# ipc-sim/IPC

Hardware: NVIDIA H100
Metric: newton_iteration_ms_assembly_ccd (lower is better)
Workload: dtype f64

## Files before the change

ipc_b200/csrc/abi.h:

```cpp
#pragma once
#include "../../include/ipcgpu.h"
#include "context.h"
#include <cstddef>
#include <string>

#define CK(call)                                                                                  \
    do {                                                                                          \
        cudaError_t e_ = (call);                                                                  \
        if (e_ != cudaSuccess) {                                                                  \
            ctx->err = std::string(#call) + ": " + cudaGetErrorString(e_);                        \
            return IPCGPU_ERR_CUDA;                                                               \
        }                                                                                         \
    } while (0)
#define REQUIRE(cond, code, msg)                                                                  \
    do {                                                                                          \
        if (!(cond)) {                                                                            \
            ctx->err = (msg);                                                                     \
            return (code);                                                                        \
        }                                                                                         \
    } while (0)
#define ALLOC(buf, count) REQUIRE((buf).reserve(count), IPCGPU_ERR_CUDA, "cudaMalloc failed for " #buf)

static inline int nblk(long long n, int b) { return (int)((n + b - 1) / b); }

enum Chain { kSerial, kStepBound, kDerivative };

inline int join_deriv(ipcgpu_ctx* ctx)
{
    if (!ctx->deriv_open) return IPCGPU_OK;
    ctx->deriv_open = false;
    CK(cudaEventRecord(ctx->ev_deriv_done, ctx->deriv));
    CK(cudaStreamWaitEvent(ctx->stream, ctx->ev_deriv_done, 0));
    return IPCGPU_OK;
}

inline int enter(ipcgpu_ctx* ctx, Chain chain)
{
    CK(cudaSetDevice(ctx->device));
    if (chain == kStepBound) return IPCGPU_OK;
    if (chain == kSerial || ctx->nranks > 1 || ctx->profiling) return join_deriv(ctx);
    if (ctx->deriv_open) return IPCGPU_OK;
    CK(cudaEventRecord(ctx->ev_deriv_fork, ctx->stream));
    CK(cudaStreamWaitEvent(ctx->deriv, ctx->ev_deriv_fork, 0));
    ctx->deriv_open = true;
    return IPCGPU_OK;
}
#define ENTER(chain)                                                                              \
    do {                                                                                          \
        int re_ = enter(ctx, (chain));                                                            \
        if (re_) return re_;                                                                      \
    } while (0)

int join_copy_stream(ipcgpu_ctx* ctx);
int fetch_iter_state(ipcgpu_ctx* ctx);
int sync_pattern_mirror(ipcgpu_ctx* ctx);
int flag_status(ipcgpu_ctx* ctx, unsigned mask);
void set_local(ipcgpu_ctx* ctx, unsigned bits, bool local);
int energy_result(ipcgpu_ctx* ctx, int slot, double* E, bool fetch = false, unsigned check = 0);
int energy_tail(ipcgpu_ctx* ctx, int slot, const double* partials, int n_partials, double scale, cudaEvent_t pe, double* E, bool fetch = false,
    unsigned check = 0);
int gradient_roundtrip_begin(ipcgpu_ctx* ctx, const double* g_in);
int gradient_roundtrip_end(ipcgpu_ctx* ctx, double* g_out);
int hessian_begin(ipcgpu_ctx* ctx, Chain chain, const double* a_inout);
int hessian_end(ipcgpu_ctx* ctx, double* a_inout, unsigned check);

int nccl_sum(ipcgpu_ctx* ctx, double* buf, size_t n, const char* what);
int nccl_sum(ipcgpu_ctx* ctx, int* buf, size_t n, const char* what);
int nccl_min_u64(ipcgpu_ctx* ctx, unsigned long long* word);
int nccl_all_gather(ipcgpu_ctx* ctx, const int4* send, int4* recv, size_t n, const char* what);
void nccl_comm_destroy(ipcgpu_ctx* ctx);

int build_maps(ipcgpu_ctx* ctx);
void owned_value_range(ipcgpu_ctx* ctx);
int ensure_offsets(ipcgpu_ctx* ctx);
int upload_dir(ipcgpu_ctx* ctx, const double* p);

int timestep_prepare(ipcgpu_ctx* ctx, ipcgpu::DynamicsArgs* p);
// ... 56 lines not shown
```

ipc_b200/csrc/api.cu:

```cuda
#include "abi.h"
#include <cstring>

using namespace ipcgpu;

int join_copy_stream(ipcgpu_ctx* ctx)
{
    if (!ctx->copy_pending) return IPCGPU_OK;
    CK(cudaEventRecord(ctx->ev_copy_join, ctx->copy));
    CK(cudaStreamWaitEvent(ctx->stream, ctx->ev_copy_join, 0));
    ctx->copy_pending = false;
    return IPCGPU_OK;
}

int fetch_iter_state(ipcgpu_ctx* ctx)
{
    {
        int rcj = join_copy_stream(ctx);
        if (rcj) return rcj;
    }
    CK(cudaMemcpyAsync(ctx->h_iter, ctx->iter.p, sizeof(IterState), cudaMemcpyDeviceToHost, ctx->stream));
    CK(cudaStreamSynchronize(ctx->stream));
    return IPCGPU_OK;
}

// ... 127 lines not shown

int hessian_begin(ipcgpu_ctx* ctx, Chain chain, const double* a_inout)
{
    REQUIRE(ctx->nnz > 0, IPCGPU_ERR_STATE, "ipcgpu_set_csr first");
    ENTER(a_inout ? kSerial : chain);
    return a_inout ? upload_values(ctx, a_inout) : IPCGPU_OK;
}
int hessian_end(ipcgpu_ctx* ctx, double* a_inout, unsigned check)
{
    if (!a_inout) return IPCGPU_OK;
    int rc = download_values(ctx, a_inout);
    if (rc || !check || (rc = fetch_iter_state(ctx))) return rc;
    return flag_status(ctx, check);
}

extern "C" {

int ipcgpu_create(int device, ipcgpu_ctx** out)
{
    if (!out) return IPCGPU_ERR_ARG;
    *out = nullptr;
    int ndev = 0;
    if (cudaGetDeviceCount(&ndev) != cudaSuccess || ndev == 0) return IPCGPU_ERR_CUDA;
    if (device < 0 || device >= ndev) return IPCGPU_ERR_ARG;
    if (cudaSetDevice(device) != cudaSuccess) return IPCGPU_ERR_CUDA;
    ipcgpu_ctx* ctx = new ipcgpu_ctx();
    ctx->device = device;
    void* hi = nullptr;
    if (cudaDeviceGetStreamPriorityRange(&ctx->prio_low, &ctx->prio_high) != cudaSuccess
        || cudaStreamCreateWithPriority(&ctx->stream, cudaStreamNonBlocking, ctx->prio_high) != cudaSuccess
        || cudaStreamCreateWithPriority(&ctx->deriv, cudaStreamNonBlocking, ctx->prio_low) != cudaSuccess
        || cudaEventCreateWithFlags(&ctx->ev_deriv_fork, cudaEventDisableTiming) != cudaSuccess
        || cudaEventCreateWithFlags(&ctx->ev_deriv_done, cudaEventDisableTiming) != cudaSuccess
        || cudaStreamCreateWithFlags(&ctx->side, cudaStreamNonBlocking) != cudaSuccess || cudaEventCreateWithFlags(&ctx->ev_inputs, cudaEventDisableTiming) != cudaSuccess
        || cudaEventCreateWithFlags(&ctx->ev_join, cudaEventDisableTiming) != cudaSuccess || cudaEventCreateWithFlags(&ctx->ev_scatter, cudaEventDisableTiming) != cudaSuccess
        || cudaMallocHost(&ctx->staging, sizeof(HostStaging)) != cudaSuccess
        || cudaMallocHost(&hi, sizeof(IterState)) != cudaSuccess || !ctx->flag.reserve(4) || !ctx->packed_scalars.reserve(kPackedScalars) || !ctx->iter.reserve(1)
        || cudaMemsetAsync(ctx->iter.p, 0, sizeof(IterState), ctx->stream) != cudaSuccess) {
        ipcgpu_destroy(ctx);
        return IPCGPU_ERR_CUDA;
    }
    ctx->h_iter = static_cast<IterState*>(hi);
    std::memset(ctx->h_iter, 0, sizeof(IterState));
    step_set(ctx->iter.p, 1.0, ctx->stream);
    *out = ctx;
    return IPCGPU_OK;
}

void ipcgpu_destroy(ipcgpu_ctx* ctx)
{
    if (!ctx) return;
    cudaSetDevice(ctx->device);
    if (ctx->side) cudaStreamSynchronize(ctx->side);
    if (ctx->deriv) cudaStreamSynchronize(ctx->deriv);
    if (ctx->copy) {
        cudaStreamSynchronize(ctx->copy);
        cudaStreamDestroy(ctx->copy);
        cudaEventDestroy(ctx->ev_copy_fork);
        cudaEventDestroy(ctx->ev_copy_join);
    }
    if (ctx->stream) cudaStreamSynchronize(ctx->stream);
    for (auto& r : ctx->graphs) {
        if (r.exec) cudaGraphExecDestroy(r.exec);
        if (r.graph) cudaGraphDestroy(r.graph);
    }
    if (ctx->ev_inputs) cudaEventDestroy(ctx->ev_inputs);
    if (ctx->ev_join) cudaEventDestroy(ctx->ev_join);
    if (ctx->ev_scatter) cudaEventDestroy(ctx->ev_scatter);
    if (ctx->side) cudaStreamDestroy(ctx->side);
    if (ctx->ev_deriv_fork) cudaEventDestroy(ctx->ev_deriv_fork);
    if (ctx->ev_deriv_done) cudaEventDestroy(ctx->ev_deriv_done);
    if (ctx->deriv) cudaStreamDestroy(ctx->deriv);
    for (cudaStream_t s : ctx->cond_streams)
        if (s) cudaStreamDestroy(s);
    for (auto& v : ctx->prof)
        for (auto& pr : v) {
            cudaEventDestroy(pr.first);
            cudaEventDestroy(pr.second);
        }
    if (ctx->timer_a) cudaEventDestroy(ctx->timer_a);
    if (ctx->timer_b) cudaEventDestroy(ctx->timer_b);
    nccl_comm_destroy(ctx);
    if (ctx->stream) cudaStreamDestroy(ctx->stream);
    if (ctx->staging) cudaFreeHost(ctx->staging);
    if (ctx->h_iter) cudaFreeHost(ctx->h_iter);
    delete ctx;
}

const char* ipcgpu_last_error(const ipcgpu_ctx* ctx) { return ctx ? ctx->err.c_str() : "null context"; }
int ipcgpu_host_alloc(void** ptr, uint64_t bytes) { return cudaMallocHost(ptr, bytes) == cudaSuccess ? IPCGPU_OK : IPCGPU_ERR_CUDA; }
int ipcgpu_host_free(void* ptr) { return cudaFreeHost(ptr) == cudaSuccess ? IPCGPU_OK : IPCGPU_ERR_CUDA; }
int ipcgpu_sync(ipcgpu_ctx* ctx)
{
    ENTER(kSerial);
    int rcj = join_copy_stream(ctx);
    if (rcj) return rcj;
    CK(cudaStreamSynchronize(ctx->stream));
    return IPCGPU_OK;
}
uint64_t ipcgpu_launch_count(const ipcgpu_ctx* ctx) { return ctx ? ctx->launches : 0; }

int ipcgpu_allreduce_grad_hess(ipcgpu_ctx* ctx, int with_gradient, int with_hessian)
{
    if (ctx->nranks <= 1) return IPCGPU_OK;
// ... 210 lines not shown
```

ipc_b200/csrc/api_contact.cu:

```cuda
#include "abi.h"
#include <algorithm>
#include <cmath>
#include <vector>

using namespace ipcgpu;

extern "C" {

int ipcgpu_set_surface(ipcgpu_ctx* ctx, int nSV, const int* SVI, int nSE, const int* SE, int nSF, const int* SF, const int* vCoDim)
{
    ENTER(kSerial);
    ++ctx->epoch;
    REQUIRE(ctx->nV > 0, IPCGPU_ERR_STATE, "ipcgpu_set_mesh first");
    REQUIRE(nSV >= 0 && nSE >= 0 && nSF >= 0 && (nSV == 0 || SVI) && (nSE == 0 || SE) && (nSF == 0 || SF), IPCGPU_ERR_ARG, "ipcgpu_set_surface: bad arguments");
    for (int i = 0; i < nSV; ++i) REQUIRE(SVI[i] >= 0 && SVI[i] < ctx->nV, IPCGPU_ERR_ARG, "SVI out of range");
    for (int i = 0; i < 2 * nSE; ++i) REQUIRE(SE[i] >= 0 && SE[i] < ctx->nV, IPCGPU_ERR_ARG, "SFEdges out of range");
    for (size_t i = 0; i < (size_t)3 * nSF; ++i) REQUIRE(SF[i] >= 0 && SF[i] < ctx->nV, IPCGPU_ERR_ARG, "SF out of range");
    ctx->nSV = nSV; ctx->nSE = nSE; ctx->nSF = nSF;
    bool ok = ctx->SVI.upload(SVI, std::max(nSV, 0), ctx->stream) && ctx->SE.upload(SE, (size_t)2 * nSE, ctx->stream) && ctx->SF.upload(SF, (size_t)3 * nSF, ctx->stream);
    REQUIRE(ok, IPCGPU_ERR_CUDA, "surface upload failed");
    ctx->has_codim = vCoDim != nullptr;
    if (vCoDim) REQUIRE(ctx->vCoDim.upload(vCoDim, ctx->nV, ctx->stream), IPCGPU_ERR_CUDA, "codim upload failed");
    CK(cudaStreamSynchronize(ctx->stream));
    ctx->h_SVI.assign(SVI, SVI + nSV);
// ... 162 lines not shown
}

int ipcgpu_ccd_stats_timing(ipcgpu_ctx* ctx, uint64_t* longest_pair_cycles, uint64_t* total_pair_cycles)
{
    if (longest_pair_cycles) *longest_pair_cycles = ctx->ccd.last_longest_cycles;
    if (total_pair_cycles) *total_pair_cycles = ctx->ccd.last_total_cycles;
    return IPCGPU_OK;
}

int ipcgpu_set_exchange_capacity(ipcgpu_ctx* ctx, int pairs_per_rank)
{
    ENTER(kSerial);
    ++ctx->epoch;
    REQUIRE(pairs_per_rank > 0, IPCGPU_ERR_ARG, "capacity must be positive");
    ctx->exchange_capacity = pairs_per_rank;
    if (ctx->surface_ready) return contact_alloc(ctx);
    return IPCGPU_OK;
}

int ipcgpu_set_pair_capacity(ipcgpu_ctx* ctx, int capacity)
{
    ENTER(kSerial);
    ++ctx->epoch;
    REQUIRE(capacity > 0, IPCGPU_ERR_ARG, "capacity must be positive");
    ctx->pair_capacity = capacity;
    if (ctx->surface_ready) return contact_alloc(ctx);
    return IPCGPU_OK;
}

int ipcgpu_constraint_set(ipcgpu_ctx* ctx, double dHat, int getPTEE, int* nC, int* nPara, int* nCand)
{
    REQUIRE(ctx->surface_ready, IPCGPU_ERR_STATE, "ipcgpu_set_surface first");
    REQUIRE(dHat > 0.0, IPCGPU_ERR_ARG, "dHat must be positive");
    ENTER(kSerial);
    int rc = contact_constraint_set(ctx, dHat, getPTEE, nC, nPara, nCand);
    ctx->lists_local = (rc == 0) && ctx->partition_contact && ctx->nranks > 1;
    ctx->cw.lists_global = false;
    if (rc == 0 && ctx->lists_local) {
        ContactWork& w = ctx->cw;
        contact_pack_lists(ctx);
        cudaEvent_t pe = ctx->prof_begin(IPCGPU_STAGE_ALLREDUCE);
        const int r = nccl_all_gather(ctx, w.xsend.p, w.xrecv.p, w.xstride, "ncclAllGather(pair lists) failed");
        ctx->prof_end(pe);
        if (r) return r;
        contact_unpack_lists(ctx);
        w.lists_global = true;
        CK(cudaGetLastError());
    }
    ctx->mark_inputs();
    return rc;
}

int ipcgpu_set_canonical_order(ipcgpu_ctx* ctx, int enable)
{
    ENTER(kSerial);
    ++ctx->epoch;
    ctx->canonical_order = enable != 0;
    return IPCGPU_OK;
}

int ipcgpu_set_contact_partition(ipcgpu_ctx* ctx, int enable)
{
    ENTER(kSerial);
    ++ctx->epoch;
    ctx->partition_contact = enable != 0;
    return IPCGPU_OK;
}
// ... 106 lines not shown
    if ((rc = sync_pattern_mirror(ctx))) return rc;
    if (changed) *changed = ctx->pat_changed_host;
    if (nnz) *nnz = ctx->nnz;
    return flag_status(ctx, 1u << FLAG_PATTERN_CAPACITY);
}

int ipcgpu_pattern_info(ipcgpu_ctx* ctx, int* changed, int64_t* nnz, uint64_t* version)
{
    REQUIRE(ctx->device_pattern, IPCGPU_ERR_STATE, "ipcgpu_enable_device_pattern first");
    ENTER(kSerial);
    int rc = sync_pattern_mirror(ctx);
    if (rc) return rc;
    if (changed) *changed = ctx->pat_changed_host;
    if (nnz) *nnz = ctx->nnz;
    if (version) *version = ctx->pat_seen_version;
    return IPCGPU_OK;
}

int ipcgpu_get_pattern(ipcgpu_ctx* ctx, int* ia, int* ja)
{
    REQUIRE(ctx->n_rows > 0, IPCGPU_ERR_STATE, "no pattern: ipcgpu_set_csr or ipcgpu_enable_device_pattern first");
    ENTER(kSerial);
    int rc = sync_pattern_mirror(ctx);
    if (rc) return rc;
    if (ia) CK(cudaMemcpyAsync(ia, ctx->ia.p, ((size_t)ctx->n_rows + 1) * sizeof(int), cudaMemcpyDeviceToHost, ctx->stream));
    if (ja) CK(cudaMemcpyAsync(ja, ctx->ja.p, (size_t)ctx->nnz * sizeof(int), cudaMemcpyDeviceToHost, ctx->stream));
    CK(cudaStreamSynchronize(ctx->stream));
    return IPCGPU_OK;
}

int ipcgpu_barrier_energy(ipcgpu_ctx* ctx, double dHat, double kappa, double* E)
{
    REQUIRE(ctx->surface_ready, IPCGPU_ERR_STATE, "ipcgpu_set_surface first");
    ENTER(kSerial);
    BarrierArgs p = barrier_args(ctx, dHat, kappa, 0);
    cudaEvent_t pe = ctx->prof_begin(IPCGPU_STAGE_BARRIER);
    barrier_energy(p, ctx->cw.bpartials.p, &ctx->iter.p->flags[FLAG_NONPOSITIVE_DISTANCE], ctx->stream);
    return energy_tail(ctx, kEnergyBarrier, ctx->cw.bpartials.p, barrier_energy_blocks(), kappa, pe, E, true, 1u << FLAG_NONPOSITIVE_DISTANCE);
}

int ipcgpu_barrier_gradient(ipcgpu_ctx* ctx, double dHat, double kappa, double* g_inout)
{
    REQUIRE(ctx->surface_ready, IPCGPU_ERR_STATE, "ipcgpu_set_surface first");
    const BarrierArgs p = barrier_args(ctx, dHat, kappa, 0);
    return gradient_call(ctx, kDerivative, g_inout, [&](cudaStream_t st) { barrier_gradient(p, ctx->g.p, st); });
}

int ipcgpu_evaluate_constraints(ipcgpu_ctx* ctx, double* val, int n)
{
    REQUIRE(ctx->surface_ready, IPCGPU_ERR_STATE, "ipcgpu_set_surface first");
    ENTER(kSerial);
    ContactWork& w = ctx->cw;
    if (w.nC < 0) {
        int rc = contact_sync_counts(ctx);
        if (rc) return rc;
    }
    REQUIRE(n == w.nC && (val || n == 0), IPCGPU_ERR_ARG, "ipcgpu_evaluate_constraints: n must be the size of the active set on this context");
    ALLOC(w.bval, (size_t)std::max(w.cap, 1));
    BarrierArgs p = barrier_args(ctx, 1.0, 1.0, 0);
    p.cs = w.act.p; p.nC = w.counters.p + 0;
    evaluate_constraints(p, w.bval.p, ctx->stream);
    ++ctx->launches;
    CK(cudaGetLastError());
    if (n) CK(cudaMemcpyAsync(val, w.bval.p, (size_t)n * sizeof(double), cudaMemcpyDeviceToHost, ctx->stream));
    CK(cudaStreamSynchronize(ctx->stream));
    return IPCGPU_OK;
}
// ... 206 lines not shown
```

ipc_b200/csrc/api_mesh.cu:

```cuda
#include "abi.h"
#include <algorithm>
#include <cmath>
#include <numeric>
#include <vector>

using namespace ipcgpu;

int build_maps(ipcgpu_ctx* ctx)
{
    const int nT = ctx->nT, nV = ctx->nV;
    const std::vector<int>& T = ctx->h_T;
    ctx->t_begin = (int)((int64_t)nT * ctx->rank / ctx->nranks);
    ctx->t_end = (int)((int64_t)nT * (ctx->rank + 1) / ctx->nranks);
    std::vector<int64_t> cum(nV + 1, 0);
    for (size_t i = 0; i < (size_t)4 * nT; ++i) ++cum[T[i] + 1];
    for (int v = 0; v < nV; ++v) cum[v + 1] += cum[v];
    auto boundary = [&](int r) -> int {
        if (r <= 0) return 0;
        if (r >= ctx->nranks) return nV;
        const int64_t target = cum[nV] * r / ctx->nranks;
        return (int)(std::lower_bound(cum.begin(), cum.end(), target) - cum.begin());
    };
    const int vb = std::min(boundary(ctx->rank), nV), ve = std::max(vb, std::min(boundary(ctx->rank + 1), nV));
    ctx->v_begin = vb;
// ... 306 lines not shown
        e_part = ctx->e_partials2.p;
    }
    elastic_grad_hess(ctx->eargs(), coef, projectSPD, need_g, need_h, ctx->gcont.p, ctx->hblk.p, st, e_part);
    ctx->hblk_valid = need_h;
    ctx->prof_end(pe);
    ++ctx->launches;
    if (with_energy) {
        pe = ctx->prof_begin(IPCGPU_STAGE_ELASTIC_ENERGY);
        reduce_sum(e_part, elastic_grad_hess_blocks(ctx->n_list), coef, &ctx->iter.p->energy[kEnergyElastic], st);
        ctx->prof_end(pe);
        ++ctx->launches;
    }
    if (need_g) {
        pe = ctx->prof_begin(IPCGPU_STAGE_GATHER_GRADIENT);
        gather_gradient(ctx->nV, ctx->inc_ptr.p, ctx->inc.p, ctx->gcont.p, ctx->has_dbc ? ctx->dbc.p : nullptr, projectDBC, 0, ctx->g.p, st);
        ctx->prof_end(pe);
        ++ctx->launches;
    }
    if (need_h) {
        pe = ctx->prof_begin(IPCGPU_STAGE_ASSEMBLE_CSR);
        assemble_csr(ctx->nOffSlots, ctx->nSlots, ctx->slot_v.p, ctx->slot_u.p, ctx->slot_off.p, ctx->con_ptr.p, ctx->con_src.p, ctx->hblk.p,
            ctx->has_dbc ? ctx->dbc.p : nullptr, projectDBC, nullptr, cleared ? 0 : 1, ctx->a.p, st);
        const double* m = (add_mass && ctx->has_mass) ? ctx->mass.p : nullptr;
        diag_mass_dbc_range(ctx->v_begin, ctx->v_end, ctx->ia.p, ctx->index_base, ctx->has_dbc ? ctx->dbc.p : nullptr, projectDBC, m, ctx->a.p, st);
        ctx->prof_end(pe);
        ctx->launches += 2;
    }
    CK(cudaGetLastError());
    return IPCGPU_OK;
}

int ipcgpu_elastic_gradient(ipcgpu_ctx* ctx, double coef, int , int projectDBC, double* g)
{
    ENTER(g ? kSerial : kDerivative);
    int rc = run_grad_hess(ctx, coef, 1, projectDBC, true, false, 0);
    return rc || !g ? rc : gradient_roundtrip_end(ctx, g);
}

int ipcgpu_elastic_hessian(ipcgpu_ctx* ctx, double coef, int , int projectSPD, int projectDBC, double* a_inout)
{
    int rc = hessian_begin(ctx, kDerivative, a_inout);
    if (rc || (rc = run_grad_hess(ctx, coef, projectSPD, projectDBC, false, true, 0))) return rc;
    return hessian_end(ctx, a_inout, 0);
}

static int elastic_derivatives(ipcgpu_ctx* ctx, double coef, int projectSPD, int projectDBC, int add_mass, bool with_energy, double* E, double* g, double* a)
{
    REQUIRE(ctx->nnz > 0, IPCGPU_ERR_STATE, "ipcgpu_set_csr first");
    ENTER(E || g || a ? kSerial : kDerivative);
    int rc = a ? sync_pattern_mirror(ctx) : 0;
    if (rc || (rc = zero_values(ctx))) return rc;
    if ((rc = run_grad_hess(ctx, coef, projectSPD, projectDBC, true, true, add_mass, with_energy, true))) return rc;
    if (ctx->nranks > 1 && (g || a)) {
        rc = ipcgpu_allreduce_grad_hess(ctx, g ? 1 : 0, a ? 1 : 0);
        if (rc) return rc;
    }
    if (g) CK(cudaMemcpyAsync(g, ctx->g.p, (size_t)3 * ctx->nV * sizeof(double), cudaMemcpyDeviceToHost, ctx->stream));
    if (a) CK(cudaMemcpyAsync(a, ctx->a.p, (size_t)ctx->nnz * sizeof(double), cudaMemcpyDeviceToHost, ctx->stream));
    if (with_energy && (rc = energy_result(ctx, kEnergyElastic, E))) return rc;
    if (!E && (g || a)) CK(cudaStreamSynchronize(ctx->stream));
    return IPCGPU_OK;
}

int ipcgpu_elastic_grad_hess(ipcgpu_ctx* ctx, double coef, int projectSPD, int projectDBC, int add_mass, double* g, double* a)
{
    return elastic_derivatives(ctx, coef, projectSPD, projectDBC, add_mass, false, nullptr, g, a);
}

int ipcgpu_elastic_energy_grad_hess(ipcgpu_ctx* ctx, double coef, int projectSPD, int projectDBC, int add_mass, double* E, double* g, double* a)
{
    return elastic_derivatives(ctx, coef, projectSPD, projectDBC, add_mass, true, E, g, a);
}

int ipcgpu_step_bound_set(ipcgpu_ctx* ctx, double alpha)
{
    REQUIRE(alpha >= 0.0, IPCGPU_ERR_ARG, "the step must be non-negative");
    ENTER(kStepBound);
    step_set(ctx->iter.p, alpha, ctx->stream);
    ++ctx->launches;
    CK(cudaGetLastError());
    return IPCGPU_OK;
}
// ... 93 lines not shown
```

ipc_b200/csrc/api_step.cu:

```cuda
#include "abi.h"
#include <cstring>
#include <vector>

using namespace ipcgpu;

template <typename F>
static cudaError_t for_each_kernel_node(cudaGraph_t top, const std::vector<cudaGraph_t>& bodies, F f)
{
    cudaError_t e = cudaSuccess;
    for (size_t b = 0; e == cudaSuccess && b <= bodies.size(); ++b) {
        cudaGraph_t g = b == 0 ? top : bodies[b - 1];
        size_t n = 0;
        e = cudaGraphGetNodes(g, nullptr, &n);
        std::vector<cudaGraphNode_t> nodes(n);
        if (e == cudaSuccess && n) e = cudaGraphGetNodes(g, nodes.data(), &n);
        for (size_t i = 0; e == cudaSuccess && i < n; ++i) {
            cudaGraphNodeType type;
            if (cudaGraphNodeGetType(nodes[i], &type) != cudaSuccess) {
                cudaGetLastError();
                continue;
            }
            if (type != cudaGraphNodeTypeKernel) continue;
            cudaKernelNodeAttrValue v;
            e = cudaGraphKernelNodeGetAttribute(nodes[i], cudaKernelNodeAttributePriority, &v);
// ... 13 lines not shown
    h.lists_global = ctx->cw.lists_global;
    h.want_cand = ctx->cw.want_cand;
    h.swept_ready = ctx->ccd.swept_ready;
    h.fr_ready = ctx->cw.fr_ready;
    h.inputs_marked = false;
    h.scatter_marked = false;
    h.nC = ctx->cw.nC; h.nP = ctx->cw.nP; h.nK = ctx->cw.nK; h.fr_host_n = ctx->cw.fr_host_n;
    h.hs_set_built = ctx->hs_set_built;
    h.hs_lag_ready = ctx->hs_lag_ready;
    return h;
}
static void apply_host_state(ipcgpu_ctx* ctx, const ipcgpu_ctx::HostState& h)
{
    ctx->local_scalars = h.local_scalars;
    ctx->lists_local = h.lists_local;
    ctx->cw.lists_global = h.lists_global;
    ctx->cw.want_cand = h.want_cand;
    ctx->ccd.swept_ready = h.swept_ready;
    ctx->cw.fr_ready = h.fr_ready;
    ctx->inputs_marked = h.inputs_marked;
    ctx->scatter_marked = h.scatter_marked;
    ctx->cw.nC = h.nC; ctx->cw.nP = h.nP; ctx->cw.nK = h.nK; ctx->cw.fr_host_n = h.fr_host_n;
    ctx->hs_set_built = h.hs_set_built;
    ctx->hs_lag_ready = h.hs_lag_ready;
}

int ipcgpu_capture_begin(ipcgpu_ctx* ctx)
{
    REQUIRE(!ctx->capturing, IPCGPU_ERR_STATE, "a capture is already in progress");
    REQUIRE(!ctx->profiling, IPCGPU_ERR_STATE, "switch the stage timers off (ipcgpu_profile(ctx, 0)) before capturing");
    ENTER(kSerial);
    ctx->inputs_marked = false;
    ctx->scatter_marked = false;
    ctx->deriv_copied = false;
    ctx->launches_at_capture = ctx->launches;
    ctx->dirty_at_capture = ctx->a_all_dirty;
    ctx->pat_pending_at_capture = ctx->pat_pending;
    ctx->pat_pending = false;
    ctx->sc_pending_at_capture = ctx->sc_pending;
    ctx->sc_pending = false;
    ctx->capture_bodies.clear();
    CK(cudaStreamBeginCapture(ctx->stream, cudaStreamCaptureModeThreadLocal));
    ctx->capturing = true;
    return IPCGPU_OK;
}

int ipcgpu_capture_end(ipcgpu_ctx* ctx, int* graph_id)
{
    REQUIRE(ctx->capturing, IPCGPU_ERR_STATE, "no capture in progress");
    REQUIRE(graph_id != nullptr, IPCGPU_ERR_ARG, "null graph id");
    ENTER(kSerial);
    {
        int rcj = join_copy_stream(ctx);
        if (rcj) return rcj;
    }
    ctx->capturing = false;
    ipcgpu_ctx::GraphRec rec;
    cudaError_t e = cudaStreamEndCapture(ctx->stream, &rec.graph);
    if (e != cudaSuccess || rec.graph == nullptr) {
        cudaGetLastError();
        ctx->err = std::string("stream capture failed (a call inside the capture synchronised or copied to the host? use NULL outputs): ") + cudaGetErrorString(e);
        return IPCGPU_ERR_CUDA;
    }
    if (ctx->deriv_copied) {
        e = for_each_kernel_node(rec.graph, ctx->capture_bodies, [&](cudaGraphNode_t node, cudaKernelNodeAttrValue v) {
            v.priority = (v.priority == ctx->prio_high) ? ctx->prio_low : ctx->prio_high;
            return cudaGraphKernelNodeSetAttribute(node, cudaKernelNodeAttributePriority, &v);
        });
        if (e != cudaSuccess) {
            cudaGraphDestroy(rec.graph);
            ctx->err = std::string("kernel node priorities: ") + cudaGetErrorString(e);
            return IPCGPU_ERR_CUDA;
        }
    }
    e = cudaGraphInstantiateWithFlags(&rec.exec, rec.graph, cudaGraphInstantiateFlagUseNodePriority);
    if (e != cudaSuccess) {
        cudaGraphDestroy(rec.graph);
        ctx->err = std::string("cudaGraphInstantiate: ") + cudaGetErrorString(e);
        return IPCGPU_ERR_CUDA;
    }
    rec.launches = ctx->launches - ctx->launches_at_capture;
    rec.epoch = ctx->epoch;
    rec.dirty_at_begin = ctx->dirty_at_capture;
    rec.updates_pattern = ctx->pat_pending;
    ctx->pat_pending = ctx->pat_pending_at_capture;
    rec.step_control = ctx->sc_pending;
    ctx->sc_pending = ctx->sc_pending_at_capture;
    rec.bodies.swap(ctx->capture_bodies);
    rec.hs = snapshot_host_state(ctx);
    ctx->launches = ctx->launches_at_capture;
    ctx->inputs_marked = false;
    ctx->scatter_marked = false;
    ctx->graphs.push_back(rec);
    *graph_id = (int)ctx->graphs.size() - 1;
    return IPCGPU_OK;
}

int ipcgpu_graph_launch(ipcgpu_ctx* ctx, int graph_id)
{
    REQUIRE(graph_id >= 0 && graph_id < (int)ctx->graphs.size() && ctx->graphs[graph_id].exec, IPCGPU_ERR_ARG, "unknown graph id");
    REQUIRE(!ctx->capturing, IPCGPU_ERR_STATE, "a capture is in progress");
    const ipcgpu_ctx::GraphRec& rec = ctx->graphs[graph_id];
    REQUIRE(rec.epoch == ctx->epoch, IPCGPU_ERR_STATE, "the scene, pattern, partition or capacities changed since this graph was captured: capture it again");
    ENTER(kSerial);
    if (ctx->a_all_dirty && !rec.dirty_at_begin)
        CK(cudaMemsetAsync(ctx->a.p, 0, (size_t)(ctx->device_pattern ? ctx->pw.nnz_cap : ctx->nnz) * sizeof(double), ctx->stream));
    CK(cudaGraphLaunch(rec.exec, ctx->stream));
    if (rec.updates_pattern) ctx->pat_pending = true;
    if (rec.step_control) ctx->sc_pending = true;
    ctx->a_all_dirty = false;
    apply_host_state(ctx, rec.hs);
    ctx->launches += rec.launches;
    return IPCGPU_OK;
}

int ipcgpu_graph_destroy(ipcgpu_ctx* ctx, int graph_id)
{
    REQUIRE(graph_id >= 0 && graph_id < (int)ctx->graphs.size(), IPCGPU_ERR_ARG, "unknown graph id");
    ENTER(kSerial);
    ipcgpu_ctx::GraphRec& rec = ctx->graphs[graph_id];
    if (rec.exec) cudaGraphExecDestroy(rec.exec);
    if (rec.graph) cudaGraphDestroy(rec.graph);
    rec.exec = nullptr;
    rec.graph = nullptr;
    return IPCGPU_OK;
// ... 43 lines not shown
{
    REQUIRE(ctx->surface_ready, IPCGPU_ERR_STATE, "ipcgpu_set_surface first");
    ENTER(kSerial);
    cudaEvent_t pe = ctx->prof_begin(IPCGPU_STAGE_HASH);
    int rc = safeguard_intersections(ctx);
    ctx->prof_end(pe);
    REQUIRE(rc == 0, rc, "intersection check launch failed");
    set_local(ctx, kLocalChecks, true);
    if (ok) {
        CK(cudaMemsetAsync(&ctx->iter.p->checks[0], 0, sizeof(int), ctx->stream));
        if ((rc = reduce_checks(ctx))) return rc;
        if ((rc = fetch_iter_state(ctx))) return rc;
        *ok = ctx->h_iter->checks[1] == 0 ? 1 : 0;
    }
    return IPCGPU_OK;
}

static int decide(ipcgpu_ctx* ctx, int op, double a, int b, cudaGraphConditionalHandle h, bool* word)
{
    step_decide(ctx->iter.p, op, a, b, (unsigned long long)h, ctx->stream);
    ++ctx->launches;
    CK(cudaGetLastError());
    if (word) {
        CK(cudaMemcpyAsync(&ctx->staging->decision, &ctx->iter.p->ls_cond, sizeof(int), cudaMemcpyDeviceToHost, ctx->stream));
        CK(cudaStreamSynchronize(ctx->stream));
        *word = ctx->staging->decision != 0;
    }
    return IPCGPU_OK;
}

}

template <typename Body>
static int cond_node(ipcgpu_ctx* ctx, bool loop, int op, double a, int b, Body body)
{
    int rc;
    if (!ctx->capturing) {
        bool go = false;
        if ((rc = decide(ctx, op, a, b, 0, &go))) return rc;
        while (go) {
            if ((rc = body())) return rc;
            if (!loop) break;
            if ((rc = decide(ctx, op, a, b, 0, &go))) return rc;
        }
        return IPCGPU_OK;
    }
    REQUIRE(ctx->cond_depth < ipcgpu_ctx::kCondDepth, IPCGPU_ERR_STATE, "conditional nodes nested too deeply");
    cudaStreamCaptureStatus cs;
    cudaGraph_t g = nullptr;
    const cudaGraphNode_t* deps = nullptr;
    size_t nd = 0;
    CK(cudaStreamGetCaptureInfo(ctx->stream, &cs, nullptr, &g, &deps, &nd));
    cudaGraphConditionalHandle h = 0;
    const cudaError_t eh = cudaGraphConditionalHandleCreate(&h, g, 0, 0);
    if (eh != cudaSuccess) {
        cudaGetLastError();
        ctx->err = std::string("conditional graph nodes need CUDA 12.4 or newer in the driver: ") + cudaGetErrorString(eh);
        return IPCGPU_ERR_CUDA;
    }
    if ((rc = decide(ctx, op, a, b, h, nullptr))) return rc;
    CK(cudaStreamGetCaptureInfo(ctx->stream, &cs, nullptr, &g, &deps, &nd));
    cudaGraphNodeParams np = {};
    np.type = cudaGraphNodeTypeConditional;
    np.conditional.handle = h;
    np.conditional.type = loop ? cudaGraphCondTypeWhile : cudaGraphCondTypeIf;
    np.conditional.size = 1;
    cudaGraphNode_t node;
    CK(cudaGraphAddNode(&node, g, deps, nd, &np));
    cudaGraph_t bg = np.conditional.phGraph_out[0];
    ctx->capture_bodies.push_back(bg);
    cudaStream_t outer = ctx->stream, inner = ctx->cond_streams[ctx->cond_depth];
    CK(cudaStreamBeginCaptureToGraph(inner, bg, nullptr, nullptr, 0, cudaStreamCaptureModeThreadLocal));
    ctx->stream = inner;
    ++ctx->cond_depth;
    ctx->inputs_marked = false;
    rc = body();
    if (!rc && loop) rc = decide(ctx, op, a, b, h, nullptr);
    --ctx->cond_depth;
    ctx->stream = outer;
    cudaGraph_t captured = nullptr;
    const cudaError_t ee = cudaStreamEndCapture(inner, &captured);
    if (rc) return rc;
    CK(ee);
    CK(cudaStreamUpdateCaptureDependencies(outer, &node, 1, cudaStreamSetCaptureDependencies));
    ctx->mark_inputs();
    return IPCGPU_OK;
}

extern "C" {

static int step_control_prepare(ipcgpu_ctx* ctx)
{
    REQUIRE(ctx->surface_ready && ctx->maps_ready, IPCGPU_ERR_STATE, "ipcgpu_set_mesh and ipcgpu_set_surface first");
    REQUIRE(ctx->nranks == 1, IPCGPU_ERR_STATE, "the CFL branch and the line search run on one rank");
    REQUIRE(ctx->dir_valid && ctx->pSize_surface, IPCGPU_ERR_STATE, "no search direction for this surface: ipcgpu_set_search_dir first");
    if (!ctx->cond_streams[0]) {
        REQUIRE(!ctx->capturing, IPCGPU_ERR_STATE, "run the CFL branch / line search once outside a capture first (it creates its streams)");
        for (cudaStream_t& s : ctx->cond_streams) CK(cudaStreamCreateWithPriority(&s, cudaStreamNonBlocking, ctx->prio_high));
    }
    return IPCGPU_OK;
}

static int step_control_status(ipcgpu_ctx* ctx, int status)
{
    if (status == IPCGPU_ERR_LINE_SEARCH)
        ctx->err = "step 0: the line search's entry state fails a safeguard (inversion / intersection), or the step bound or the entry step is 0";
    else if (status == IPCGPU_ERR_NONPOSITIVE_DISTANCE)
        ctx->err = "a line-search trial has a constraint with d <= 0 (the reference exits here, Optimizer.cpp:3296-3306)";
    return status;
// ... 208 lines not shown
```

ipc_b200/csrc/constraint.cu:

```cuda
#include "broadphase.cuh"
#include "abi.h"
#include <cub/cub.cuh>

namespace ipcgpu {

DEV void grow(Box& b, V3 x)
{
    b.lo[0] = fmin(b.lo[0], x.x); b.hi[0] = fmax(b.hi[0], x.x);
    b.lo[1] = fmin(b.lo[1], x.y); b.hi[1] = fmax(b.hi[1], x.y);
    b.lo[2] = fmin(b.lo[2], x.z); b.hi[2] = fmax(b.hi[2], x.z);
}
DEV Box empty_box()
{
    Box b;
    for (int a = 0; a < 3; ++a) { b.lo[a] = 1e300; b.hi[a] = -1e300; }
    return b;
}

__global__ void __launch_bounds__(256) k_boxes(SurfArgs s, int prim, Box* __restrict__ boxes, unsigned long long* __restrict__ bounds)
{
    const int n = prim == 0 ? s.nSV : (prim == 1 ? s.nSE : s.nSF);
    const int i = blockIdx.x * blockDim.x + threadIdx.x;
    Box b = empty_box();
    double ext = 0.0;
// ... 804 lines not shown
    const SurfArgs s = surf_args(ctx);
    const double radius = sqrt(dHat);
    cudaEvent_t pe = ctx->prof_begin(IPCGPU_STAGE_HASH);
    int rc;
    if ((rc = boxes_and_grid(ctx, radius, true))) return rc;
    ctx->prof_end(pe);

    pe = ctx->prof_begin(IPCGPU_STAGE_CONSTRAINT_SET);
    CK(cudaMemsetAsync(w.counters.p, 0, 16 * sizeof(int), st));
    CsOut out;
    out.act = w.act.p; out.nAct = w.counters.p + 0; out.capAct = w.cap;
    out.dup = w.dup.p; out.nDup = w.counters.p + 1; out.capDup = w.cap;
    out.para = w.para.p; out.para_e = w.para_e.p; out.nPara = w.counters.p + 2; out.capPara = w.cap;
    out.cand = w.cand.p; out.nCand = w.counters.p + 3; out.capCand = 4 * w.cap;
    out.overflow = w.counters.p + 4;
    const SortedGrid tg = tri_grid(ctx), eg = edge_grid(ctx);
    int v0 = 0, v1 = s.nSV, e0 = 0, e1 = s.nSE;
    if (ctx->partition_contact && ctx->nranks > 1) {
        v0 = (int)((long long)s.nSV * ctx->rank / ctx->nranks); v1 = (int)((long long)s.nSV * (ctx->rank + 1) / ctx->nranks);
        e0 = (int)((long long)s.nSE * ctx->rank / ctx->nranks); e1 = (int)((long long)s.nSE * (ctx->rank + 1) / ctx->nranks);
    }
    unsigned* nPairs = reinterpret_cast<unsigned*>(w.counters.p + 8);
    PairOut ppt{ w.bp_pairs.p, nPairs, (unsigned)w.bp_cap, w.counters.p + 4 }, pee{ w.bp_pairs.p + w.bp_cap, nPairs + 1, (unsigned)w.bp_cap, w.counters.p + 4 };
    if (v1 > v0 && s.nSF > 0) {
        cell_pairs_pt(w.grid.p, vertex_grid(ctx), tg, s, radius, s.nSF + s.nSE + v0, s.nSF + s.nSE + v1, ppt, st);
        k_classify_pt<<<kSMs * 8, 128, 0, st>>>(s, ppt.pairs, ppt.n, ppt.cap, dHat, wantCand, out);
        ctx->launches += 2;
    }
    if (e1 > e0 && s.nSE > 1) {
        cell_pairs_ee(w.grid.p, eg, s, radius, s.nSF + e0, s.nSF + e1, pee, st);
        k_classify_ee<<<kSMs * 8, 128, 0, st>>>(s, pee.pairs, pee.n, pee.cap, dHat, wantCand, out);
        ctx->launches += 2;
    }
    const bool hashed_merge = ctx->nV < (1 << 21) - 2;
    if (hashed_merge) {
        CK(cudaMemsetAsync(w.skey.p, 0xff, (size_t)w.dup_tab * sizeof(unsigned long long), st));
        CK(cudaMemsetAsync(w.sidx.p, 0, (size_t)w.dup_tab * sizeof(int), st));
        k_dup_insert<<<kSMs * 2, 256, 0, st>>>(w.counters.p + 1, w.cap, w.dup.p, w.skey.p, w.sidx.p, w.dup_tab - 1, w.counters.p + 4);
        k_dup_emit<<<nblk(w.dup_tab, 256), 256, 0, st>>>(w.dup_tab, w.skey.p, w.sidx.p, w.act.p, w.counters.p + 0, w.cap, w.counters.p + 4);
        ctx->launches += 2;
    }
    w.want_cand = wantCand != 0;
    w.nC = w.nP = w.nK = -1;
    const bool need_host = !hashed_merge || ctx->canonical_order || nC || nPara || nCand;
    if (need_host) {
        int* h = ctx->staging->contact;
        if (!hashed_merge) {
            CK(cudaMemcpyAsync(h, w.counters.p, 8 * sizeof(int), cudaMemcpyDeviceToHost, st));
            CK(cudaStreamSynchronize(st));
            const int nDup = std::min(h[1], w.cap);
            if (nDup > 0) {
                if ((rc = sort_lex(ctx, w.dup.p, nullptr, nDup, w.tmp4.p, nullptr))) return rc;
                k_merge_dups<<<nblk(nDup, 256), 256, 0, st>>>(nDup, w.dup.p, w.act.p, w.counters.p + 0, w.cap, w.counters.p + 4);
                ++ctx->launches;
            }
        }
        if ((rc = contact_sync_counts(ctx))) return rc;
        if (ctx->canonical_order) {
            if ((rc = sort_lex(ctx, w.act.p, nullptr, w.nC, w.tmp4.p, nullptr))) return rc;
            if ((rc = sort_lex(ctx, w.para.p, w.para_e.p, w.nP, w.tmp4.p, w.tmp2.p))) return rc;
            if (wantCand && (rc = sort_int2(ctx, w.cand.p, w.nK, w.tmp2.p))) return rc;
        }
    }
    k_publish_counts<<<1, 32, 0, st>>>(w.counters.p, wantCand, ctx->iter.p);
    ++ctx->launches;
    ctx->prof_end(pe);
// ... 6 lines not shown
```

ipc_b200/csrc/context.h:

```cpp
#pragma once
#include "kernels.h"
#include "broadphase_types.h"
#include <cuda_runtime.h>
#include <cstdint>
#include <cstring>
#include <string>
#include <vector>

namespace ipcgpu {

template <typename T>
struct DevBuf {
    T* p = nullptr;
    size_t n = 0;
    ~DevBuf() { release(); }
    void release()
    {
        if (p) cudaFree(p);
        p = nullptr;
        n = 0;
    }
    bool reserve(size_t count)
    {
        if (count <= n) return true;
// ... 79 lines not shown
};

constexpr int kMultilevelMax = 8;
struct MultilevelWork {
    DevBuf<double> box, inv, R, Y, part, chunk;
    DevBuf<unsigned> code, code_sorted;
    DevBuf<int> id, order, rank;
    DevBuf<unsigned char> sort_tmp, fixed;
    bool built = false;
    int levels = 0;
    long long domains[kMultilevelMax] = {};
    size_t tile_off[kMultilevelMax] = {}, tiles = 0;
    bool smem_opted = false;
};

struct HostStaging {
    double scalar;
    int count;
    int contact[16];
    double pcg[8];
    double pSize;
    int decision;
    int hs_count[2];
};

}

struct ipcgpu_ctx {
    int device = 0;
    cudaStream_t stream = nullptr;
    cudaStream_t deriv = nullptr;
    cudaEvent_t ev_deriv_fork = nullptr, ev_deriv_done = nullptr;
    bool deriv_open = false, deriv_copied = false;
    int prio_low = 0, prio_high = 0;
    cudaStream_t deriv_stream() const { return deriv_open ? deriv : stream; }
    cudaStream_t side = nullptr;
    cudaStream_t copy = nullptr;
    cudaEvent_t ev_copy_fork = nullptr, ev_copy_join = nullptr;
    bool copy_pending = false;
    cudaEvent_t ev_inputs = nullptr, ev_join = nullptr, ev_scatter = nullptr;
    bool scatter_marked = false;
    bool inputs_marked = false;
    void mark_inputs()
    {
        inputs_marked = (cudaEventRecord(ev_inputs, stream) == cudaSuccess);
    }
    std::string err;
    uint64_t launches = 0;

    int rank = 0, nranks = 1;
    void* nccl_comm = nullptr;
    int v_begin = 0, v_end = 0, n_list = 0;
    ipcgpu::DevBuf<int> tet_list;
    long long a_begin = 0, a_end = 0;

    ipcgpu::DevBuf<ipcgpu::IterState> iter;
    ipcgpu::IterState* h_iter = nullptr;
    double pSize = 0.0;
    bool dir_valid = false, pSize_surface = false;
    unsigned local_scalars = 0;
    bool a_all_dirty = false;
    std::vector<int> h_ia;

    int nV = 0, nT = 0, energy = 0;
    int t_begin = 0, t_end = 0;
    ipcgpu::DevBuf<double> V, Vsaved, Vrest, Ainv, vol, mu, lam, mass, Vprev, xtilde;
// ... 116 lines not shown
```

Baseline: 2.814.

## Fork elastic derivative work earlier so it overlaps contact detection

Adds a 'front' chain and an elastic-inputs event so elastic gradient/Hessian kernels can fork onto the derivative stream as soon as their inputs are ready, rather than waiting behind the constraint-set and barrier energy work on the main stream. The event is re-recorded after the broad-phase classification so elastic work runs concurrently with the dedup/merge and barrier kernels. The intent is to hide elastic assembly latency behind contact detection. It adds stream-ordering state that must be reset at graph capture and in step bodies, which risks subtle ordering bugs. A profiling script is included.

```diff
diff --git a/ipc_b200/csrc/abi.h b/ipc_b200/csrc/abi.h
--- a/ipc_b200/csrc/abi.h
+++ b/ipc_b200/csrc/abi.h
@@ -23,7 +23,7 @@
 
 static inline int nblk(long long n, int b) { return (int)((n + b - 1) / b); }
 
-enum Chain { kSerial, kStepBound, kDerivative };
+enum Chain { kSerial, kFront, kStepBound, kDerivative, kElastic };
 
 inline int join_deriv(ipcgpu_ctx* ctx)
 {
@@ -34,15 +34,42 @@
     return IPCGPU_OK;
 }
 
+inline int advance_elastic_mark(ipcgpu_ctx* ctx)
+{
+    if (ctx->elastic_marked) CK(cudaEventRecord(ctx->ev_elastic_inputs, ctx->stream));
+    return IPCGPU_OK;
+}
+
 inline int enter(ipcgpu_ctx* ctx, Chain chain)
 {
     CK(cudaSetDevice(ctx->device));
     if (chain == kStepBound) return IPCGPU_OK;
-    if (chain == kSerial || ctx->nranks > 1 || ctx->profiling) return join_deriv(ctx);
-    if (ctx->deriv_open) return IPCGPU_OK;
+    if (chain == kSerial || ctx->nranks > 1 || ctx->profiling || (chain == kFront && ctx->step_body > 0)) {
+        ctx->elastic_marked = false;
+        return join_deriv(ctx);
+    }
+    if (chain == kFront) {
+        int rc = join_deriv(ctx);
+        if (rc) return rc;
+        if (!ctx->elastic_marked) {
+            CK(cudaEventRecord(ctx->ev_elastic_inputs, ctx->stream));
+            ctx->elastic_marked = true;
+        }
+        return IPCGPU_OK;
+    }
+    if (chain == kElastic && (ctx->deriv_open || ctx->elastic_marked)) {
+        if (!ctx->deriv_open) {
+            CK(cudaStreamWaitEvent(ctx->deriv, ctx->ev_elastic_inputs, 0));
+            ctx->deriv_open = true;
+            ctx->deriv_at_tail = false;
+        }
+        return IPCGPU_OK;
+    }
+    if (ctx->deriv_open && ctx->deriv_at_tail) return IPCGPU_OK;
     CK(cudaEventRecord(ctx->ev_deriv_fork, ctx->stream));
     CK(cudaStreamWaitEvent(ctx->deriv, ctx->ev_deriv_fork, 0));
     ctx->deriv_open = true;
+    ctx->deriv_at_tail = true;
     return IPCGPU_OK;
 }
 #define ENTER(chain)                                                                              \
diff --git a/ipc_b200/csrc/api.cu b/ipc_b200/csrc/api.cu
--- a/ipc_b200/csrc/api.cu
+++ b/ipc_b200/csrc/api.cu
@@ -183,6 +183,7 @@
         || cudaStreamCreateWithPriority(&ctx->deriv, cudaStreamNonBlocking, ctx->prio_low) != cudaSuccess
         || cudaEventCreateWithFlags(&ctx->ev_deriv_fork, cudaEventDisableTiming) != cudaSuccess
         || cudaEventCreateWithFlags(&ctx->ev_deriv_done, cudaEventDisableTiming) != cudaSuccess
+        || cudaEventCreateWithFlags(&ctx->ev_elastic_inputs, cudaEventDisableTiming) != cudaSuccess
         || cudaStreamCreateWithFlags(&ctx->side, cudaStreamNonBlocking) != cudaSuccess || cudaEventCreateWithFlags(&ctx->ev_inputs, cudaEventDisableTiming) != cudaSuccess
         || cudaEventCreateWithFlags(&ctx->ev_join, cudaEventDisableTiming) != cudaSuccess || cudaEventCreateWithFlags(&ctx->ev_scatter, cudaEventDisableTiming) != cudaSuccess
         || cudaMallocHost(&ctx->staging, sizeof(HostStaging)) != cudaSuccess
@@ -221,6 +222,7 @@
     if (ctx->side) cudaStreamDestroy(ctx->side);
     if (ctx->ev_deriv_fork) cudaEventDestroy(ctx->ev_deriv_fork);
     if (ctx->ev_deriv_done) cudaEventDestroy(ctx->ev_deriv_done);
+    if (ctx->ev_elastic_inputs) cudaEventDestroy(ctx->ev_elastic_inputs);
     if (ctx->deriv) cudaStreamDestroy(ctx->deriv);
     for (cudaStream_t s : ctx->cond_streams)
         if (s) cudaStreamDestroy(s);
diff --git a/ipc_b200/csrc/api_contact.cu b/ipc_b200/csrc/api_contact.cu
--- a/ipc_b200/csrc/api_contact.cu
+++ b/ipc_b200/csrc/api_contact.cu
@@ -218,7 +218,7 @@
 {
     REQUIRE(ctx->surface_ready, IPCGPU_ERR_STATE, "ipcgpu_set_surface first");
     REQUIRE(dHat > 0.0, IPCGPU_ERR_ARG, "dHat must be positive");
-    ENTER(kSerial);
+    ENTER(nC || nPara || nCand ? kSerial : kFront);
     int rc = contact_constraint_set(ctx, dHat, getPTEE, nC, nPara, nCand);
     ctx->lists_local = (rc == 0) && ctx->partition_contact && ctx->nranks > 1;
     ctx->cw.lists_global = false;
@@ -391,7 +391,7 @@
 int ipcgpu_barrier_energy(ipcgpu_ctx* ctx, double dHat, double kappa, double* E)
 {
     REQUIRE(ctx->surface_ready, IPCGPU_ERR_STATE, "ipcgpu_set_surface first");
-    ENTER(kSerial);
+    ENTER(E ? kSerial : kFront);
     BarrierArgs p = barrier_args(ctx, dHat, kappa, 0);
     cudaEvent_t pe = ctx->prof_begin(IPCGPU_STAGE_BARRIER);
     barrier_energy(p, ctx->cw.bpartials.p, &ctx->iter.p->flags[FLAG_NONPOSITIVE_DISTANCE], ctx->stream);
diff --git a/ipc_b200/csrc/api_mesh.cu b/ipc_b200/csrc/api_mesh.cu
--- a/ipc_b200/csrc/api_mesh.cu
+++ b/ipc_b200/csrc/api_mesh.cu
@@ -362,14 +362,14 @@
 
 int ipcgpu_elastic_gradient(ipcgpu_ctx* ctx, double coef, int , int projectDBC, double* g)
 {
-    ENTER(g ? kSerial : kDerivative);
+    ENTER(g ? kSerial : kElastic);
     int rc = run_grad_hess(ctx, coef, 1, projectDBC, true, false, 0);
     return rc || !g ? rc : gradient_roundtrip_end(ctx, g);
 }
 
 int ipcgpu_elastic_hessian(ipcgpu_ctx* ctx, double coef, int , int projectSPD, int projectDBC, double* a_inout)
 {
-    int rc = hessian_begin(ctx, kDerivative, a_inout);
+    int rc = hessian_begin(ctx, kElastic, a_inout);
     if (rc || (rc = run_grad_hess(ctx, coef, projectSPD, projectDBC, false, true, 0))) return rc;
     return hessian_end(ctx, a_inout, 0);
 }
@@ -377,7 +377,7 @@
 static int elastic_derivatives(ipcgpu_ctx* ctx, double coef, int projectSPD, int projectDBC, int add_mass, bool with_energy, double* E, double* g, double* a)
 {
     REQUIRE(ctx->nnz > 0, IPCGPU_ERR_STATE, "ipcgpu_set_csr first");
-    ENTER(E || g || a ? kSerial : kDerivative);
+    ENTER(E || g || a ? kSerial : kElastic);
     int rc = a ? sync_pattern_mirror(ctx) : 0;
     if (rc || (rc = zero_values(ctx))) return rc;
     if ((rc = run_grad_hess(ctx, coef, projectSPD, projectDBC, true, true, add_mass, with_energy, true))) return rc;
diff --git a/ipc_b200/csrc/api_step.cu b/ipc_b200/csrc/api_step.cu
--- a/ipc_b200/csrc/api_step.cu
+++ b/ipc_b200/csrc/api_step.cu
@@ -69,6 +69,7 @@
     ENTER(kSerial);
     ctx->inputs_marked = false;
     ctx->scatter_marked = false;
+    ctx->elastic_marked = false;
     ctx->deriv_copied = false;
     ctx->launches_at_capture = ctx->launches;
     ctx->dirty_at_capture = ctx->a_all_dirty;
@@ -128,6 +129,7 @@
     ctx->launches = ctx->launches_at_capture;
     ctx->inputs_marked = false;
     ctx->scatter_marked = false;
+    ctx->elastic_marked = false;
     ctx->graphs.push_back(rec);
     *graph_id = (int)ctx->graphs.size() - 1;
     return IPCGPU_OK;
@@ -237,6 +239,16 @@
 }
 
 template <typename Body>
+static int in_step_body(ipcgpu_ctx* ctx, Body& body)
+{
+    ++ctx->step_body;
+    const int rc = body();
+    --ctx->step_body;
+    ctx->elastic_marked = false;
+    return rc;
+}
+
+template <typename Body>
 static int cond_node(ipcgpu_ctx* ctx, bool loop, int op, double a, int b, Body body)
 {
     int rc;
@@ -244,7 +256,8 @@
         bool go = false;
         if ((rc = decide(ctx, op, a, b, 0, &go))) return rc;
         while (go) {
-            if ((rc = body())) return rc;
+            rc = in_step_body(ctx, body);
+            if (rc) return rc;
             if (!loop) break;
             if ((rc = decide(ctx, op, a, b, 0, &go))) return rc;
         }
@@ -279,7 +292,7 @@
     ctx->stream = inner;
     ++ctx->cond_depth;
     ctx->inputs_marked = false;
-    rc = body();
+    rc = in_step_body(ctx, body);
     if (!rc && loop) rc = decide(ctx, op, a, b, h, nullptr);
     --ctx->cond_depth;
     ctx->stream = outer;
diff --git a/ipc_b200/csrc/constraint.cu b/ipc_b200/csrc/constraint.cu
--- a/ipc_b200/csrc/constraint.cu
+++ b/ipc_b200/csrc/constraint.cu
@@ -860,6 +860,7 @@
         k_classify_ee<<<kSMs * 8, 128, 0, st>>>(s, pee.pairs, pee.n, pee.cap, dHat, wantCand, out);
         ctx->launches += 2;
     }
+    if ((rc = advance_elastic_mark(ctx))) return rc;
     const bool hashed_merge = ctx->nV < (1 << 21) - 2;
     if (hashed_merge) {
         CK(cudaMemsetAsync(w.skey.p, 0xff, (size_t)w.dup_tab * sizeof(unsigned long long), st));
diff --git a/ipc_b200/csrc/context.h b/ipc_b200/csrc/context.h
--- a/ipc_b200/csrc/context.h
+++ b/ipc_b200/csrc/context.h
@@ -135,6 +135,9 @@
     cudaStream_t deriv = nullptr;
     cudaEvent_t ev_deriv_fork = nullptr, ev_deriv_done = nullptr;
     bool deriv_open = false, deriv_copied = false;
+    cudaEvent_t ev_elastic_inputs = nullptr;
+    bool elastic_marked = false, deriv_at_tail = false;
+    int step_body = 0;
     int prio_low = 0, prio_high = 0;
     cudaStream_t deriv_stream() const { return deriv_open ? deriv : stream; }
     cudaStream_t side = nullptr;
diff --git a/profiles/fork_timing.py b/profiles/fork_timing.py
--- /dev/null
+++ b/profiles/fork_timing.py
@@ -0,0 +1,138 @@
+#!/usr/bin/env python
+import argparse
+import json
+import os
+import subprocess
+import sys
+import tempfile
+import time
+
+import numpy as np
+
+ROOT = os.path.dirname(os.path.dirname(os.path.abspath(__file__)))
+sys.path.insert(0, ROOT)
+
+import bench
+
+
+def card():
+    try:
+        return subprocess.run(["nvidia-smi", "--query-gpu=name,power.limit,clocks.max.sm", "--format=csv,noheader"], capture_output=True, text=True,
+                              timeout=30).stdout.strip()
+    except (OSError, subprocess.SubprocessError) as e:
+        return f"nvidia-smi unavailable: {e}"
+
+
+def main():
+    ap = argparse.ArgumentParser()
+    ap.add_argument("--tets", type=int, default=1_000_000)
+    ap.add_argument("--scene", default="c5", choices=["c5", "pile"])
+    ap.add_argument("--res", type=int, default=10)
+    ap.add_argument("--iters", type=int, default=5)
+    ap.add_argument("--warmup", type=int, default=5)
+    ap.add_argument("--trace", default=None, help="also keep the chrome trace here")
+    args = ap.parse_args()
+
+    import torch
+    from torch.profiler import ProfilerActivity, profile
+    from ipc_b200 import lib as L
+
+    torch.cuda.init()
+    m, info = bench.build_scene(args)
+    ctx = L.Context(0)
+    ctx.set_mesh(m.V_rest_soa, m.T_soa, m.restTriInv, m.vol, m.mu, m.lam, m.mass, m.dbc, m.energy)
+    ctx.set_surface(m.SVI, m.SFEdges, m.SF_soa, m.vCoDim)
+    ctx.set_state(m.V_soa)
+    dHat, hvox = info["dHat"], m.avgEdgeLen / 3.0
+    err_vf, err_ee = L.Context.ti_error(m.V_soa, m.nV, None)
+    mm, pa, pe, _ = ctx.constraint_set(dHat, 1)
+    ia, ja = m.csr_pattern(1, extra_pairs=bench.contact_pattern_pairs(m, mm, pa, pe))
+    ctx.set_csr(ia, ja, 1)
+    ctx.set_contact_partition(1)
+    ctx.set_canonical_order(0)
+    ctx.set_search_dir(info["p"])
+
+    def enqueue_iteration():
+        ctx.constraint_set(dHat, 1, fetch=False, sizes=False)
+        ctx.barrier_energy(dHat, bench.KAPPA, want=False)
+        ctx.elastic_energy_grad_hess(bench.DT2, 1, 1, 1, None, None)
+        ctx.barrier_gradient(dHat, bench.KAPPA, None)
+        ctx.barrier_hessian(dHat, bench.KAPPA, 1, None)
+        ctx.allreduce_grad_hess(1, 0)
+        ctx.step_bound_set(1.0)
+        ctx.inversion_step(None, 0.2, None)
+        ctx.ccd_partial(None, bench.TI_TOL, err_vf, err_ee, None)
+        ctx.hash_build_swept(None, None, hvox)
+        ctx.ccd_full(bench.TI_TOL, err_vf, err_ee, None)
+
+    for _ in range(args.warmup):
+        enqueue_iteration()
+        ctx.fetch_iteration()
+    ctx.capture_begin()
+    enqueue_iteration()
+    graph = ctx.capture_end()
+    for _ in range(args.warmup):
+        ctx.graph_launch(graph)
+        ctx.fetch_iteration()
+    ctx.sync()
+
+    with profile(activities=[ProfilerActivity.CUDA]) as prof:
+        for _ in range(args.iters):
+            ctx.graph_launch(graph)
+            it = ctx.fetch_iteration()
+            assert it.status == 0, it.status
+            time.sleep(0.005)
+        ctx.sync()
+    path = args.trace or os.path.join(tempfile.mkdtemp(), "fork_timing.json")
+    prof.export_chrome_trace(path)
+    with open(path) as f:
+        ev = [e for e in json.load(f)["traceEvents"] if e.get("ph") == "X" and e.get("cat") in ("kernel", "gpu_memset", "gpu_memcpy")]
+    ev.sort(key=lambda e: e["ts"])
+    iters, cur = [], []
+    for e in ev:
+        if cur and e["ts"] - max(c["ts"] + c["dur"] for c in cur) > 1000.0:
+            iters.append(cur)
+            cur = []
+        cur.append(e)
+    if cur:
+        iters.append(cur)
+
+    def short(name):
+        name = name.split("(")[0].replace("void ", "")
+        return name.split("::")[-1].split("<")[0]
+
+    print("card:", card())
+    print(f"{'iter':>4} {'elastic start':>13} {'elastic end':>11} {'assemble start':>14} {'assemble end':>12} {'last scatter start':>18} "
+          f"{'last scatter end':>16} {'full CCD end':>12} {'span':>8}")
+    per_kernel = {}
+    need = ("k_elastic_grad_hess", "k_assemble_csr", "k_barrier_hessian_scatter", "k_ccd_commit")
+    for i, evs in enumerate(iters):
+        kern = [e for e in evs if e["cat"] == "kernel"]
+        names = {short(e["name"]) for e in kern}
+        if not all(k in names for k in need):
+            print(f"{i:>4} (not an iteration: {len(evs)} activities, {sorted(names)[:8]})")
+            continue
+        t0 = min(e["ts"] for e in kern)
+        t1 = max(e["ts"] + e["dur"] for e in kern)
+        by = {}
+        for e in kern:
+            by.setdefault(short(e["name"]), []).append(e)
+            per_kernel.setdefault(short(e["name"]), []).append(e["dur"])
+
+        def se(name, which=0):
+            e = by[name][which]
+            return e["ts"] - t0, e["ts"] + e["dur"] - t0
+
+        el, asm, sc = se("k_elastic_grad_hess"), se("k_assemble_csr"), se("k_barrier_hessian_scatter", -1)
+        ccd_end = by["k_ccd_commit"][-1]["ts"] + by["k_ccd_commit"][-1]["dur"] - t0
+        print(f"{i:>4} {el[0]:>13.1f} {el[1]:>11.1f} {asm[0]:>14.1f} {asm[1]:>12.1f} {sc[0]:>18.1f} {sc[1]:>16.1f} {ccd_end:>12.1f} {t1 - t0:>8.1f}")
+    n = max(1, sum(1 for evs in iters if any(short(e["name"]) == "k_elastic_grad_hess" for e in evs)))
+    print(f"\nper-kernel device time over {len(iters)} iterations (median us per launch, launches per iteration, us per iteration):")
+    for k in sorted(per_kernel, key=lambda k: -sum(per_kernel[k])):
+        d = per_kernel[k]
+        print(f"  {k:<32} {float(np.median(d)):>9.1f} {len(d) / n:>5.0f} {sum(d) / n:>9.1f}")
+    ctx.close()
+
+
+if __name__ == "__main__":
+    main()
```

Result: faster. 2.707 (median of 6 runs) (-3.8%).
